# Complexity-ML/complexity-tokenizer

Hardware: AMD Instinct MI355X
Metric: MB/s raw UTF-8 encoded (encode_batch), 50k ByteLevel BPE, 1/2/4/8 MI355X (higher is better)
Workload: dtype u8

## Files before the change

### complexity-tokenizer_amd/complexity_tokenizer/__init__.py

```python
from __future__ import annotations

import ctypes
import gc
import os

import numpy as np

from . import _native as _n
from . import _fast

__version__ = "0.3.3"
__all__ = ["Tokenizer", "Trainer", "Encoding", "BatchEncoding", "PanicException", "UnsupportedConfigError",
           "DeviceError", "__version__"]


class PanicException(BaseException):
    """Raised where the reference raises pyo3_runtime.PanicException (a Rust panic), e.g. a
    merge rank that indexes past the list of valid merges (reference src/bpe.rs:141)."""


class UnsupportedConfigError(NotImplementedError):
    """tokenizer.json selects a component outside the ByteLevel-BPE encode path."""


# ... 209 lines not shown
            buf = ctypes.create_string_buffer(1024)
            rc = _n.lib.ctok_special_token(self._h, i, buf, 1024, ctypes.byref(n), ctypes.byref(tid))
            if rc != _n.CTOK_OK:
                _raise(rc)
            if n.value > 1024:
                buf = ctypes.create_string_buffer(n.value)
                _n.lib.ctok_special_token(self._h, i, buf, n.value, ctypes.byref(n), ctypes.byref(tid))
            out[buf.raw[:n.value].decode("utf-8")] = int(tid.value)
        return out

    def num_piece_added_tokens(self) -> int:
        return int(_n.lib.ctok_num_piece_added_tokens(self._h))

    @property
    def table_props(self) -> dict:
        tp = _n.TableProps()
        rc = _n.lib.ctok_get_table_props(self._h, int(self.device), ctypes.byref(tp))
        if rc != _n.CTOK_OK:
            _raise(rc)
        return {k: None if getattr(tp, k) < 0 else bool(getattr(tp, k)) for k, _ in tp._fields_}

    def encode_packed(self, text: np.ndarray, off: np.ndarray, timing: bool = False):
        text = np.ascontiguousarray(text, dtype=np.uint8)
        off = np.ascontiguousarray(off, dtype=np.uint64)
        n_docs = len(off) - 1
        if n_docs < 0:
            raise ValueError("offsets must hold n_docs + 1 entries")
        n_bytes = int(off[-1]) if n_docs >= 0 else 0
        if len(text) < n_bytes:
            raise ValueError("text shorter than offsets[-1]")
        cap = int(n_bytes + n_docs + 16)
        while True:
            ids = np.empty(max(cap, 1), dtype=np.uint32)
            tok_off = np.empty(n_docs + 1, dtype=np.uint64)
            ex = self._host_exec(timing)
# ... 395 lines not shown
```

### complexity-tokenizer_amd/complexity_tokenizer/_native.py

```python
from __future__ import annotations

import ctypes
import os

_HERE = os.path.dirname(os.path.abspath(__file__))
LIB_PATH = os.environ.get("CTOK_LIB", os.path.join(_HERE, "libctok.so"))

if not os.path.exists(LIB_PATH):
    raise ImportError(
        "complexity_tokenizer: native library not found at %s -- build it with "
        "`make -C complexity-tokenizer_amd/csrc` (or `python -c 'import __graft_entry__ as g; g.build()'`)" % LIB_PATH)


def _share_torch_hip_runtime():
    if os.environ.get("CTOK_NO_TORCH_HIP"):
        return
    try:
        import importlib.util
        spec = importlib.util.find_spec("torch")
    except (ImportError, ValueError):
        return
    if spec is None or not spec.origin:
        return
    path = os.path.join(os.path.dirname(spec.origin), "lib", "libamdhip64.so")
# ... 68 lines not shown

class PadOpts(ctypes.Structure):
    _fields_ = [("flags", ctypes.c_uint32), ("pad_id", ctypes.c_uint32), ("max_length", ctypes.c_uint64)]


class Tables(ctypes.Structure):
    _fields_ = [("vocab", ctypes.c_char_p), ("vocab_off", ctypes.c_void_p), ("vocab_id", ctypes.c_void_p),
                ("n_vocab", ctypes.c_uint64), ("merge_left", ctypes.c_void_p), ("merge_right", ctypes.c_void_p),
                ("n_merges", ctypes.c_uint64), ("added", ctypes.c_char_p), ("added_off", ctypes.c_void_p),
                ("added_id", ctypes.c_void_p), ("added_flags", ctypes.c_void_p), ("n_added", ctypes.c_uint64),
                ("nfc", ctypes.c_int), ("add_prefix_space", ctypes.c_int)]


class TableProps(ctypes.Structure):
    _fields_ = [(k, ctypes.c_int) for k in ("narrow", "compact", "short_packed", "ids16", "dev_narrow",
                                            "dev_short_packed", "last_rec16", "last_wire16")]


class TrainerConfig(ctypes.Structure):
    _fields_ = [("vocab_size", ctypes.c_uint64), ("min_frequency", ctypes.c_uint32),
                ("min_word_length", ctypes.c_uint64), ("inl_alpha", ctypes.c_float), ("inl_beta", ctypes.c_float),
                ("inl_gate", ctypes.c_float), ("inl_mu_target", ctypes.c_float),
                ("inl_velocity_max", ctypes.c_float), ("inl_beta_max", ctypes.c_float),
                ("special", ctypes.c_char_p), ("special_off", ctypes.POINTER(ctypes.c_uint64)),
                ("n_special", ctypes.c_uint64), ("device", ctypes.c_int)]


class TrainerCountStats(ctypes.Structure):
    _fields_ = [("pieces", ctypes.c_uint64), ("words", ctypes.c_uint64), ("unique_words", ctypes.c_uint64),
                ("chunks", ctypes.c_uint64), ("host_chunks", ctypes.c_uint64), ("rerun_chunks", ctypes.c_uint64),
                ("bytes_d2h", ctypes.c_uint64), ("ms_device", ctypes.c_double), ("ms_host", ctypes.c_double)]
# ... 67 lines not shown
```

### complexity-tokenizer_amd/csrc/ctok_host.cpp

```cpp
#include <emmintrin.h>
#include <sched.h>
#include <hip/hip_runtime.h>

#include <algorithm>
#include <atomic>
#include <chrono>
#include <cstdio>
#include <cstring>
#include <exception>
#include <fstream>
#include <functional>
#include <map>
#include <memory>
#include <mutex>
#include <sstream>
#include <thread>
#include <string>
#include <string_view>
#include <unordered_map>
#include <unordered_set>
#include <vector>

#include "../../include/ctok.h"
#include "ctok_internal.h"
// ... 1326 lines not shown
  tb.comp_val = ds->comp_val.p;
  tb.n_comp = CT_COMP_N;
  tb.bytemap_alnum = ds->alnum.p;
  tb.at_bytes = ds->at_bytes.p;
  tb.at_off = ds->at_off.p;
  tb.at_id = ds->at_id.p;
  tb.at_flags = ds->at_flags.p;
  tb.n_at = (uint32_t)t->at_id.size();
  tb.proper = (t->proper && !getenv("CTOK_FORCE_IMPROPER")) ? 1 : 0;
  tb.compact = t->compact ? 1 : 0;
  tb.narrow = (t->narrow && !getenv("CTOK_FORCE_WIDE_SLOTS")) ? 1 : 0;
  {
    const char* pk = getenv("CTOK_SHORT_PACKED");
    tb.short_packed = (tb.narrow && t->short_packed && !(pk && atoi(pk) == 0)) ? 1 : 0;
  }
  tb.all_bytes = std::all_of(t->byte2id, t->byte2id + 256, [](int32_t v) { return v >= 0; }) ? 1 : 0;
  tb.dbg = getenv("CTOK_DBG_MODE") ? (uint32_t)atoi(getenv("CTOK_DBG_MODE")) : 0;
  DeviceState* r = ds.get();
  t->devs[device] = std::move(ds);
  return r;
}

bool debug_sync() {
  static int v = -1;
  if (v < 0) v = getenv("CTOK_DEBUG_SYNC") ? 1 : 0;
  return v == 1;
}

#define STEP(name, x)                                                                    \
  do {                                                                                   \
// ... 336 lines not shown
    ds->lw_pos.ensure(n_long + 8);
    ds->lwn.ensure(n_long + 8);
    ds->scan_tmp2.ensure(scan_tmp_elems(n_long + 1) + 64);
    w.long_pos = ds->long_pos.p;
    w.lw_pos = ds->lw_pos.p;
    STEP("long_prep", launch_long_prep(w, tb, ds->side, n_long, ds->lwn.p, (uint32_t*)ds->scan_tmp2.p,
                                       ds->scan_tmp2.cap * 2));
    HIPTRY(hipMemcpyAsync((void*)tot, ds->long_pos.p + n_long, 4, hipMemcpyDeviceToHost, ds->side));
    HIPTRY(hipMemcpyAsync((void*)(tot + 1), ds->lw_pos.p + n_long, 4, hipMemcpyDeviceToHost, ds->side));
    HIPTRY(hipEventRecord(ds->ev_tot, ds->side));
  }
  const uint32_t c3n = seg_cnt[kCtrC3Count];
  const bool c3_sparse = c3n != 0 && c3n <= c3_limit && c3n <= w.c3_max;
  const char* ov_var = getenv("CTOK_OVERLAP");
  const int overlap = ov_var ? atoi(ov_var) : kOverlapDefault;
  const bool mid_side = overlap >= 1 && seg_cnt[0] == 0;
  ds->last_mid_side = mid_side;
  STEP("bpe_mid", launch_bpe_class(w, tb, 2, mid_side ? ds->side : s, lx(8, 10)));
  if (c3_sparse) STEP("bpe_c3_sparse", launch_c3_sparse(w, tb, c3n, s, lx(-1, 9)));
  else STEP("bpe_c3", launch_bpe_class(w, tb, 4, s, lx(-1, 9)));
  if (!spec_fail1 && n_long) {
    for (;;) {
      const hipError_t e = hipEventQuery(ds->ev_tot);
      if (e == hipSuccess) break;
      if (e != hipErrorNotReady) throw_err(CTOK_E_DEVICE, std::string("hipEventQuery: ") + hipGetErrorString(e));
    }
    const bool any_gmem = tot[1] != 0;
    ds->lids.ensure((uint64_t)tot[0] + 64);
    ds->lw.ensure(4 * (uint64_t)tot[1] + 64);
    w.lids = ds->lids.p;
    w.lw = ds->lw.p;
    STEP("bpe_long", launch_bpe_long(w, tb, ds->side, n_long, seg_cnt[kCtrAnyC3] != 0 && !c3_sparse, any_gmem));
  }
  if (n_long || mid_side) {
    HIPTRY(hipEventRecord(ds->ev_join, ds->side));
    HIPTRY(hipStreamWaitEvent(s, ds->ev_join, 0));
  }
  const bool dropped_pass = tb.n_at == 0 && !tb.all_bytes;
  STEP("bpe_dropped", launch_bpe_class(w, tb, 3, s, lx(5, -1)));
  static const bool copy_res = getenv("CTOK_COPY_RESULTS") != nullptr;
  w.host_res = copy_res ? nullptr : ds->host_dev;
  STEP("emit", launch_emit(w, d_ids, ids_cap, d_tok_off, s, st != nullptr, seg_cnt[kCtrEmptyDocs] != 0,
                           lx(3, -1), lx(-1, 6)));
  if (!w.host_res) {
    HIPTRY(hipMemcpyAsync(ds->host, d_tok_off + n_docs, 8, hipMemcpyDeviceToHost, s));
    HIPTRY(hipMemcpyAsync(ds->host + 1, ds->counters.p, kNumCounters * 4, hipMemcpyDeviceToHost, s));
  }
  Laps laps;
  int lap[11];
  if (tm) {
    hipEvent_t* e = ds->ev;
    const bool passes = tb.n_at == 0;
    lap[0] = laps.add(e[0], e[1]);
    lap[1] = laps.add(e[7], e[1]);
    lap[2] = laps.add(e[1], e[2]);
    lap[3] = !passes ? -1 : mid_side ? laps.add(e[2], e[10]) : laps.add(e[8], e[10]);
    lap[4] = passes ? laps.add(e[2], e[9]) : -1;
    lap[5] = laps.add(e[1], e[2]);
    lap[6] = passes ? laps.add(e[1], e[10]) : -1;
    lap[7] = passes ? laps.add(e[1], e[9]) : -1;
    lap[8] = laps.add(e[1], e[dropped_pass ? 5 : 3]);
    lap[9] = laps.add(e[3], e[6]);
    lap[10] = laps.add(e[0], e[6]);
  }
  HP(5);
  spin_sync(ds, s, [&] { laps.poll(); });
  HP(6);
  laps.finish();
  HP(7);
  uint64_t ntok = ((volatile uint64_t*)ds->host)[0];
  if (w.wgrec) {
    std::vector<uint64_t> r(kWgRecWords);
    HIPTRY(hipMemcpy(r.data(), w.wgrec, kWgRecWords * 8, hipMemcpyDeviceToHost));
    uint64_t t0 = ~0ull;
// ... 656 lines not shown
int ctok_special_token(const ctok* t, uint64_t i, char* buf, size_t cap, size_t* len, uint32_t* id) {
  if (!t || !len || !id) return fail(CTOK_E_ARG, "null argument");
  if (i >= t->special.size()) return fail(CTOK_E_ARG, "index out of range");
  const auto& e = t->special[i];
  *len = e.first.size();
  *id = e.second;
  if (buf && cap) memcpy(buf, e.first.data(), std::min(cap, e.first.size()));
  return CTOK_OK;
}

uint64_t ctok_num_piece_added_tokens(const ctok* t) { return t ? t->at_id.size() : 0; }

int ctok_get_table_props(const ctok* tc, int device, ctok_table_props* out) {
  if (!tc || !out) return fail(CTOK_E_ARG, "null argument");
  ctok* t = const_cast<ctok*>(tc);
  *out = ctok_table_props{t->narrow, t->compact, t->short_packed, t->ids16, -1, -1, -1, -1};
  std::lock_guard<std::mutex> lk(t->dev_mu);
  auto it = t->devs.find(device);
  if (it != t->devs.end()) {
    const DeviceState& ds = *it->second;
    out->dev_narrow = (int)ds.t.narrow;
    out->dev_short_packed = (int)ds.t.short_packed;
    out->last_rec16 = ds.last_rec16;
    out->last_wire16 = ds.last_wire16;
  }
  return CTOK_OK;
}

int ctok_piece_can_contain(const uint8_t* raw, size_t len) {
  if (!raw && len) return fail(CTOK_E_ARG, "null argument");
  return can_occur_in_piece(std::string((const char*)raw, len)) ? 1 : 0;
}

uint64_t ctok_ids_bound(const ctok*, uint64_t n_bytes, uint64_t n_docs) { return 3 * n_bytes + n_docs + 16; }

int ctok_device_count(void) {
  int n = 0;
  if (hipGetDeviceCount(&n) != hipSuccess) return 0;
  return n;
// ... 566 lines not shown
```

### complexity-tokenizer_amd/csrc/ctok_internal.h

```cpp
#pragma once
#include <hip/hip_runtime.h>

#include <cstdint>

namespace ctok_dev {

constexpr uint64_t kEmpty = ~0ull;
constexpr uint32_t kIdBits = 21;
constexpr uint64_t kKeyMask = (1ull << 42) - 1;
constexpr uint32_t kNoRank = 0x3FFFFFu;
constexpr uint32_t kMaxId = (1u << kIdBits) - 2;
constexpr uint32_t kPanicVal = kNoRank - 1;

constexpr uint32_t kErrPanic = 1u;

constexpr int kTileWords = 62;
constexpr int kTile = kTileWords * 64;
constexpr int kTileSlots = 4096;
constexpr int kSegWaves = 4;
constexpr int kSegUnroll = 4;
constexpr int kShortMax = 32;
constexpr int kMedMax = 64;
constexpr uint32_t kCap0 = kTile, kCap1 = (kTile + 8) / 9, kCap2 = (kTile + 16) / 17, kCap3 = (kTile + 32) / 33;
constexpr uint32_t kCap0Lean = 1040;
constexpr int kNumClasses = 4;
constexpr int kNumCounters = 32;
constexpr int kC3Shards = 64;
constexpr int kCounterWords = kNumCounters + kC3Shards;
__host__ __device__ constexpr int ctr_stat(int c) { return c < 3 ? 6 + 2 * c : 16; }
__host__ __device__ constexpr int ctr_chunk(int c) { return c < 3 ? 13 + c : 18; }
constexpr int kCtrAnyMid = 19;
constexpr int kCtrAnyC3 = 20;
constexpr int kCtrEmptyDocs = 21;
constexpr int kCtrC3Count = 22;
constexpr int kCtrC3Take = 23;
constexpr uint32_t kC3SparseDefault = 65536;
constexpr uint32_t kWgRecWords = 4 * 1024 * 4;
constexpr int kOverlapDefault = 1;
constexpr int kCtrSink = 31;
constexpr int kCtrOverflow = 25;
constexpr int kCtrLongIds = 26;
constexpr int kCtrLwWords = 27;
constexpr int kCtrRounds = 29;
constexpr int kLhBuckets = 65;
constexpr int kLhHist = 0, kLhScan = 80, kLhFill = 160, kLhTake = 240, kLhWords = 320;
__host__ __device__ inline uint32_t long_bucket(uint32_t n) { return n > 4096 ? 0u : 64u - (n - 1) / 64; }
__host__ __device__ inline uint32_t list_entry(uint32_t sl, uint32_t o, uint32_t n) { return sl | (o << 12) | (n << 24); }
__host__ __device__ inline uint32_t ent_len(uint32_t e) { return (e >> 24) & 127u; }
__host__ __device__ inline uint32_t ent_ord(uint32_t e) { return (e >> 12) & 0xFFFu; }
__host__ __device__ inline uint32_t long_ord(uint64_t e) { return (uint32_t)(e >> 32) & 0xFFFu; }
__host__ __device__ inline uint32_t long_len(uint64_t e) { return (uint32_t)(e >> 44) & 0x7FFFFu; }

// ... 84 lines not shown
  const uint32_t* comp_val;
  uint32_t n_comp;
  const uint8_t* bytemap_alnum;
  const uint8_t* at_bytes;
  const uint32_t* at_off;
  const uint32_t* at_id;
  const uint8_t* at_flags;
  uint32_t n_at;
  uint32_t proper;
  const uint32_t* eager;
  uint32_t window;
  const uint32_t* wmeta;
  uint32_t compact;
  uint32_t narrow;
  uint32_t short_packed;
  uint32_t dbg;
  uint32_t all_bytes;
};

struct Work {
  const uint8_t* text;
  uint32_t n_bytes;
  const uint64_t* doc_off;
  uint32_t n_docs;
  uint32_t* tfirst;
  uint32_t* pbits;
  uint32_t n_words;
  uint32_t n_tiles;
  uint32_t n_cus;
  uint32_t nfc_watch;
  uint32_t* nfc_bits;
  uint32_t mid_wide;
  uint32_t short_wgs;
// ... 147 lines not shown
```

### complexity-tokenizer_amd/csrc/kernels.hip

```cpp
#include <hip/hip_ext.h>
#include <hip/hip_runtime.h>

#include <algorithm>
#include <mutex>
#include <type_traits>

#include "ctok_internal.h"
#include "merge16_hd.h"
#include "seg_lane.h"

namespace ctok_dev {

#define HIPCHK(x) do { hipError_t e_ = (x); if (e_ != hipSuccess) return e_; } while (0)

template <typename F, typename... A>
static void launch_lx(const Lx& x, F k, dim3 grid, dim3 block, uint32_t lds, hipStream_t s, A... a) {
  if (x.start || x.stop)
    hipExtLaunchKernelGGL(k, grid, block, lds, s, x.start, x.stop, 0u, a...);
  else
    hipLaunchKernelGGL(k, grid, block, lds, s, a...);
}

constexpr uint32_t kNone = 0xFFFFFFFFu;
constexpr uint32_t kDead = 0xFFFFFFFFu;
// ... 1213 lines not shown
__device__ __forceinline__ void lds8_store_packed(const uint32_t (&T)[8], const uint32_t (&R)[8], lds_u32* s_key,
                                                  lds_u16* s_tok) {
  if constexpr (K0 < K1) {
    s_key[K0 * NT + threadIdx.x] = m16::lds8_key<K0>(R);
    s_tok[K0 * NT + threadIdx.x] = (uint16_t)m16::half<K0>(T);
    lds8_store_packed<K0 + 1, K1, NT>(T, R, s_key, s_tok);
  }
}
template <int K0, int K1>
__device__ __forceinline__ void store_packed_ids(const uint32_t (&T)[8], uint32_t m, uint32_t* out) {
  if constexpr (K0 < K1) {
    if ((uint32_t)K0 < m) out[K0] = m16::half<K0>(T);
    store_packed_ids<K0 + 1, K1>(T, m, out);
  }
}

template <uint32_t SORTCAP, int KT = 64>
struct PassLds {
  uint32_t pre[KT + 1], tsum[KT], tbase[KT], stat[2], bcnt[4], bfill[4], chunk, take, next;
  uint16_t perm[SORTCAP];
};

template <int N, bool COMPACT, bool HOT, uint32_t NT, uint32_t SORTCAP, bool L8 = false, int KT = 64, bool PK = false,
          typename Load>
__device__ __forceinline__ void class_pass(const Work& w, const Tables& t, const PairLds& P, const int32_t* s_b2id,
                                           PassLds<SORTCAP, KT>& S, bool& loaded, Load&& load,
                                           lds_u32* s_key = nullptr, lds_u16* s_tok = nullptr) {
  using LC = LdsClass<N>;
  constexpr int K = KT;
  static_assert(KT <= (int)NT, "a thread per chunk tile");
  const uint32_t tid = threadIdx.x;
  uint32_t* err = &w.counters[2];
  const uint32_t* list = class_list<N>(w);
  const uint32_t cap = class_cap<N>(w);
  const uint32_t* counts = w.tcls + (size_t)LC::cls * w.n_tiles;
  uint32_t st_bytes = 0, st_ids = 0;
  if (tid < 2) S.stat[tid] = 0;
  constexpr uint32_t blo = N == 8 ? 1 : N / 2 + 1, bw = N == 64 ? 8 : N == 32 ? 4 : 2;
  auto bucket = [&](uint32_t n) { return min(3u, (n - blo) / bw); };
  __syncthreads();
  uint32_t take = 1;
  const uint32_t U = w.unit;
  for (;;) {
    if (tid == 0) {
      S.chunk = atomicAdd(&w.counters[ctr_chunk(LC::cls)], take);
// ... 44 lines not shown
      }
      __syncthreads();
    }
    auto entry = [&](uint32_t i, uint32_t& kt) {
      const uint32_t q = sorted ? (uint32_t)S.perm[i] : i;
      kt = tile_of<K>(S.pre, q);
      return list[(size_t)(c0 + kt) * cap + (q - S.pre[kt])];
    };
    auto start_of = [&](uint32_t e, uint32_t kt) { return (c0 + kt) * kTile + (e & 0xFFFu); };
    auto body = [&](uint32_t e, uint32_t kt, const uint32_t* wv, auto&& hook) {
        const uint32_t tile = c0 + kt;
        const uint32_t s = tile * kTile + (e & 0xFFFu);
        const uint32_t o = ent_ord(e);
        const uint32_t n = ent_len(e);
        if constexpr (PK) {
          static_assert(N == 16 && L8 && COMPACT, "the packed tier is the 9..16 B pass's, ahead of merge_lds8, on compact tables");
          uint32_t T[8], R[8], bytes[N];
          bool missing = false;
#pragma unroll
          for (int k = 0; k < N; k++) bytes[k] = byte_of(wv[k >> 2], k);
#pragma unroll
          for (int d = 0; d < 8; d++) {
            const int32_t i0 = s_b2id[bytes[2 * d]], i1 = s_b2id[bytes[2 * d + 1]];
            missing |= (((uint32_t)(2 * d) < n) & (i0 < 0)) | (((uint32_t)(2 * d + 1) < n) & (i1 < 0));
            T[d] = m16::pack2((uint32_t)i0, (uint32_t)i1);
          }
          if (missing) {
            hook();
            const uint32_t mi = atomicAdd(&w.counters[4], 1u);
            if (mi < w.mid_cap)
              w.mid_list[mi] = (uint64_t)s | ((uint64_t)o << 32) | ((uint64_t)n << 48);
            else
              atomicOr(&w.counters[kCtrOverflow], 1u);
            return;
          }
          {
            uint32_t v[N];
#pragma unroll
            for (int k = 0; k < N - 1; k++) v[k] = t.pair0[(bytes[k] << 8) | bytes[k + 1]];
            v[N - 1] = kNoRank;
#pragma unroll
            for (int k = 0; k < N - 1; k++) v[k] = (uint32_t)k + 1 < n ? v[k] : kNoRank;
#pragma unroll
            for (int d = 0; d < 8; d++) R[d] = m16::pack2(v[2 * d], v[2 * d + 1]);
          }
          uint32_t m = n;
          Lookup16<HOT> lk{t, P, err};
          const bool more = m16::tier(T, R, m, 8u, lk);
          hook();
          uint32_t pos = 0;
          auto out_of = [&](uint32_t mm) {
            pos = atomicAdd(&S.tsum[kt], mm);
            return w.scratch + (size_t)tile * kTileSlots + pos;
          };
          if (more) {
            lds8_store_packed<0, 8, NT>(T, R, s_key, s_tok);
            m = merge_lds8_run<COMPACT, HOT, NT>(t, P, m, s_key, s_tok, err, out_of);
          } else {
            store_packed_ids<0, N>(T, m, out_of(m));
          }
          CTOK_CHECK_REC(m >= 1 && m <= n && pos + m <= (uint32_t)kTileSlots && o < (uint32_t)kTileSlots,
                         "[ctok check] packed class pass tile %u: record m=%u n=%u pos=%u ordinal=%u\n", tile, m, n, pos, o);
          w.mrec[(size_t)tile * kTileSlots + o] = rec_short(m, pos);
          st_bytes += n;
          st_ids += m;
          return;
        }
        uint32_t tk[N], rk[N];
        bool missing = false;
        {
#pragma unroll
          for (int k = 0; k < N; k++) {
            const int32_t id = s_b2id[byte_of(wv[k >> 2], k)];
            missing |= ((uint32_t)k < n) & (id < 0);
            tk[k] = (uint32_t)id;
          }
        }
// ... 67 lines not shown
      };
      constexpr int kPw = N / 4;
      uint32_t e0 = 0, kt0 = 0, e1 = 0, kt1 = 0;
      uint32_t d0[kPw + 1], sh0 = 0;
#pragma unroll
      for (int k = 0; k <= kPw; k++) d0[k] = 0;
      const uint32_t last = (w.n_bytes - 1) & ~3u;
      auto issue_words = [&](uint32_t s) {
        const uint32_t a0 = s & ~3u;
#pragma unroll
        for (int k = 0; k <= kPw; k++) d0[k] = *reinterpret_cast<const uint32_t*>(w.text + min(a0 + 4 * k, last));
        sh0 = s & 3u;
      };
      auto hook = [&]() {
        static_assert(kPw <= 8, "hook operands");
        if constexpr (kPw == 2) asm volatile("" ::"v"(d0[0]), "v"(d0[1]), "v"(d0[2]), "v"(e1));
        else if constexpr (kPw == 4)
          asm volatile("" ::"v"(d0[0]), "v"(d0[1]), "v"(d0[2]), "v"(d0[3]), "v"(d0[4]), "v"(e1));
        else
          asm volatile("" ::"v"(d0[0]), "v"(d0[1]), "v"(d0[2]), "v"(d0[3]), "v"(d0[4]), "v"(d0[5]), "v"(d0[6]),
                       "v"(d0[7]), "v"(d0[8]), "v"(e1));
      };
      uint32_t b0 = take();
      uint32_t b1 = b0 < E ? take() : E;
      if (b0 + lane < E) {
        e0 = entry(b0 + lane, kt0);
        issue_words(start_of(e0, kt0));
      }
      if (b1 + lane < E) e1 = entry(b1 + lane, kt1);
      hook();
      while (b0 < E) {
        const uint32_t i = b0 + lane;
        const uint32_t b2 = b1 < E ? take() : E;
        const uint32_t e = e0, kt = kt0;
        uint32_t wv[kPw];
#pragma unroll
        for (int k = 0; k < kPw; k++) wv[k] = __builtin_amdgcn_alignbyte(d0[k + 1], d0[k], sh0);
        e0 = e1;
        kt0 = kt1;
        if (b1 + lane < E) issue_words(start_of(e0, kt0));
        if (b2 + lane < E) e1 = entry(b2 + lane, kt1);
        b0 = b1;
        b1 = b2;
        if (i < E) body(e, kt, wv, hook);
        else hook();
      }
    }
    tile_share_flush<K>(w, c0, tb1, S.tsum, S.tbase, LC::cls);
    const uint32_t units = (w.n_tiles + U - 1) / U, next = S.chunk + S.take;
    const uint32_t share = next < units ? (units - next) / gridDim.x : 0u;
    take = min(min((uint32_t)K / U, max(1u, share)), N <= 16 ? 64u : max(1u, (2 * NT * S.take + E) / (E + 1)));
    __syncthreads();
  }
#pragma unroll
  for (int o = 32; o > 0; o >>= 1) {
    st_bytes += (uint32_t)__shfl_xor((int)st_bytes, o, 64);
    st_ids += (uint32_t)__shfl_xor((int)st_ids, o, 64);
  }
  if ((tid & 63) == 0) {
    atomicAdd(&S.stat[0], st_bytes);
// ... 8 lines not shown
}


#ifndef CTOK_SHORT_NT
#define CTOK_SHORT_NT 1024
#endif
#ifndef CTOK_SHORT_SORTCAP
#define CTOK_SHORT_SORTCAP 7168
#endif
template <bool NARROW> struct ShortCfg {
  static constexpr uint32_t NT = NARROW ? CTOK_SHORT_NT : 1024;
  static constexpr uint32_t SORTCAP = NARROW ? CTOK_SHORT_SORTCAP : kSortCap;
};
constexpr int kShortKT = 64;

template <bool COMPACT, bool NARROW, bool PK16 = false>
__global__ __launch_bounds__(1024) void k_bpe_short(Work w, Tables t, uint32_t passes) {
  static_assert((NARROW && COMPACT) || !PK16, "the packed tier needs the narrow tables and compact values");
  if (w.report && blockIdx.x == 0 && threadIdx.x < 64) write_report(w);
  if (spec_failed(w)) return;
  constexpr uint32_t NT = ShortCfg<NARROW>::NT;
  extern __shared__ __attribute__((aligned(16))) uint4 s_img[];
  __shared__ int32_t s_b2id[256];
  __shared__ PassLds<ShortCfg<NARROW>::SORTCAP, kShortKT> S;
  __shared__ uint32_t s_key[NARROW ? 8 * NT : 1];
  __shared__ uint16_t s_tok[NARROW ? 8 * NT : 1];
  const uint32_t tid = threadIdx.x;
  const uint4* img = NARROW ? t.lds16_image : t.lds_image;
  auto load = [&] {
    for (uint32_t i = tid; i < kLdsImageBytes / 16; i += NT) s_img[i] = img[i];
    for (uint32_t i = tid; i < 256; i += NT) s_b2id[i] = t.byte2id[i];
  };
  bool loaded = false;
  const PairLds P{(const lds_u64*)s_img, (const lds_u32*)(s_img + kHotBuckets)};
  lds_u32* sk = (lds_u32*)s_key;
  lds_u16* st = (lds_u16*)s_tok;
  WgRec::begin(w.wgrec, 0);
  if (passes & 1u)
    class_pass<8, COMPACT, true, NT, ShortCfg<NARROW>::SORTCAP, NARROW, kShortKT>(w, t, P, s_b2id, S, loaded, load, sk, st);
  if (passes & 2u)
    class_pass<16, COMPACT, true, NT, ShortCfg<NARROW>::SORTCAP, NARROW, kShortKT, PK16>(w, t, P, s_b2id, S, loaded, load, sk, st);
  WgRec::end(w.wgrec, 0, loaded ? 1u : 0u);
}


template <bool COMPACT, bool NARROW>
__device__ __forceinline__ uint32_t merge_wave64(const Tables& t, const PairLds& P, uint32_t& tok, uint32_t rk,
                                                 uint64_t& lv, uint32_t* err) {
  const uint32_t lane = threadIdx.x & 63;
  for (;;) {
    const uint32_t best = wave_min_full_u32((rk << 6) | lane);
    const uint32_t r = best >> 6, bi = best & 63u;
    if (r == kNoRank) break;
    const uint32_t nid = COMPACT ? r : uni(t.rank_newid[r]);
    const uint64_t right = lv & ~((2ull << bi) - 1ull);
    const uint32_t p = (uint32_t)__builtin_ctzll(right);
// ... 82 lines not shown
  WgRec::begin(w.wgrec, 3);
  extern __shared__ __attribute__((aligned(16))) uint4 s_dyn[];
  __shared__ int32_t s_b2id[256];
  const uint32_t tid = threadIdx.x;
  const uint4* img = NARROW ? t.lds16_image : t.lds_image;
  for (uint32_t i = tid; i < kLdsImageBytes / 16; i += 64 * kSparseWaves) s_dyn[i] = img[i];
  for (uint32_t i = tid; i < 256; i += 64 * kSparseWaves) s_b2id[i] = t.byte2id[i];
  __syncthreads();
  const PairLds P{(const lds_u64*)s_dyn, (const lds_u32*)(s_dyn + kHotBuckets)};
  sparse_c3<COMPACT, NARROW>(w, t, P, s_b2id, n);
  __syncthreads();
  WgRec::end(w.wgrec, 3, 1);
}


template <int CLS> struct MidCfg { static constexpr int KT = 256; };

template <bool COMPACT, int CLS, bool NARROW, uint32_t NT = 512>
__global__ __launch_bounds__(NT) void k_bpe_mid(Work w, Tables t) {
  if (spec_failed(w)) return;
  constexpr int KT = MidCfg<CLS>::KT;
  extern __shared__ __attribute__((aligned(16))) uint4 s_img[];
  __shared__ int32_t s_b2id[256];
  __shared__ PassLds<kSortCap, KT> S;
  __shared__ uint32_t s_key[NARROW ? 8 * NT : 1];
  __shared__ uint16_t s_tok[NARROW ? 8 * NT : 1];
  if constexpr (CLS == 2) WgRec::begin(w.wgrec, 1);
  if (w.counters[CLS == 2 ? kCtrAnyMid : kCtrAnyC3] == 0) {
    if constexpr (CLS == 2) WgRec::end(w.wgrec, 1, 0);
    return;
  }
  __shared__ uint32_t s_left;
  if (threadIdx.x == 0)
    s_left = (uint64_t)__atomic_load_n(&w.counters[ctr_chunk(CLS)], __ATOMIC_RELAXED) * w.unit < w.n_tiles;
  __syncthreads();
  if (!s_left) {
    if constexpr (CLS == 2) WgRec::end(w.wgrec, 1, 0);
    return;
  }
  const uint32_t tid = threadIdx.x;
  const uint4* img = NARROW ? t.lds16_image : t.lds_image;
  for (uint32_t i = tid; i < kLdsImageBytes / 16; i += NT) s_img[i] = img[i];
  for (uint32_t i = tid; i < 256; i += NT) s_b2id[i] = t.byte2id[i];
  bool loaded = true;
  const PairLds P{(const lds_u64*)s_img, (const lds_u32*)(s_img + kHotBuckets)};
  class_pass<CLS == 2 ? 32 : 64, COMPACT, true, NT, kSortCap, NARROW, KT>(w, t, P, s_b2id, S, loaded, [] {},
                                                                         (lds_u32*)s_key, (lds_u16*)s_tok);
  if constexpr (CLS == 2) WgRec::end(w.wgrec, 1, 1);
}

struct LdsAttr {
  std::mutex mu;
  uint64_t done = 0;
};
static hipError_t lds_attr_once(LdsAttr& a, const void* fn, size_t bytes) {
  int dev = 0;
  HIPCHK(hipGetDevice(&dev));
  const uint64_t bit = dev < 64 ? 1ull << dev : 0ull;
  std::lock_guard<std::mutex> lk(a.mu);
  if (a.done & bit) return hipSuccess;
  HIPCHK(hipFuncSetAttribute(fn, hipFuncAttributeMaxDynamicSharedMemorySize, (int)bytes));
  a.done |= bit;
  return hipSuccess;
}

template <bool C, int CLS, bool NW>
static hipError_t launch_mid_t(const Work& w, const Tables& t, hipStream_t s, const Lx& x) {
  static LdsAttr attr;
  HIPCHK(lds_attr_once(attr, (const void*)k_bpe_mid<C, CLS, NW>, kLdsImageBytes));
  if (!w.n_tiles) return hipSuccess;
  const uint32_t grid = min((w.n_tiles + w.unit - 1) / w.unit, w.n_cus);
  if constexpr (CLS == 2) {
    if (w.mid_wide) {
      static LdsAttr attr768;
      HIPCHK(lds_attr_once(attr768, (const void*)k_bpe_mid<C, CLS, NW, 768>, kLdsImageBytes));
      launch_lx(x, k_bpe_mid<C, CLS, NW, 768>, grid, 768, kLdsImageBytes, s, w, t);
      return hipGetLastError();
    }
  }
  launch_lx(x, k_bpe_mid<C, CLS, NW>, grid, 512, kLdsImageBytes, s, w, t);
  return hipGetLastError();
}
template <bool C, int CLS>
static hipError_t launch_mid(const Work& w, const Tables& t, hipStream_t s, const Lx& x = {}) {
  return t.narrow ? launch_mid_t<C, CLS, true>(w, t, s, x) : launch_mid_t<C, CLS, false>(w, t, s, x);
}

template <bool C, bool NW, bool PK = false>
static hipError_t launch_short_t(const Work& w, const Tables& t, hipStream_t s, const Lx& x) {
  static LdsAttr attr;
  HIPCHK(lds_attr_once(attr, (const void*)k_bpe_short<C, NW, PK>, kLdsImageBytes));
  if (!w.n_tiles) return hipSuccess;
  const uint32_t grid = min((w.n_tiles + w.unit - 1) / w.unit, w.short_wgs ? min(w.short_wgs, w.n_cus) : w.n_cus);
  if (t.dbg == 30) {
    k_bpe_short<C, NW, PK><<<grid, ShortCfg<NW>::NT, kLdsImageBytes, s>>>(w, t, 1u);
    k_bpe_short<C, NW, PK><<<grid, ShortCfg<NW>::NT, kLdsImageBytes, s>>>(w, t, 2u);
  } else {
    launch_lx(x, k_bpe_short<C, NW, PK>, grid, ShortCfg<NW>::NT, kLdsImageBytes, s, w, t, 3u);
  }
  return hipGetLastError();
}
template <bool C>
static hipError_t launch_short(const Work& w, const Tables& t, hipStream_t s, const Lx& x) {
  if constexpr (C) {
    if (t.narrow && t.short_packed) return launch_short_t<true, true, true>(w, t, s, x);
  }
  return t.narrow ? launch_short_t<C, true>(w, t, s, x) : launch_short_t<C, false>(w, t, s, x);
}

template <bool C, bool NW>
static hipError_t launch_sparse_t(const Work& w, const Tables& t, uint32_t n_pieces, hipStream_t s, const Lx& x) {
  static LdsAttr attr;
  HIPCHK(lds_attr_once(attr, (const void*)k_bpe_sparse<C, NW>, kLdsImageBytes));
  const uint32_t grid = std::max(1u, std::min((n_pieces + kSparseWaves - 1) / kSparseWaves, w.n_cus));
  launch_lx(x, k_bpe_sparse<C, NW>, grid, 64 * kSparseWaves, kLdsImageBytes, s, w, t, n_pieces);
  return hipGetLastError();
}

hipError_t launch_c3_sparse(const Work& w, const Tables& t, uint32_t n_pieces, hipStream_t s, Lx x) {
// ... 1944 lines not shown
```

### include/ctok.h

```cpp
#ifndef CTOK_H
#define CTOK_H

#include <stddef.h>
#include <stdint.h>

#ifdef __cplusplus
extern "C" {
#endif

typedef struct ctok ctok;

enum {
  CTOK_OK = 0,
  CTOK_E_IO = -1,
  CTOK_E_PARSE = -2,
  CTOK_E_UNSUPPORTED = -3,
  CTOK_E_ARG = -4,
  CTOK_E_CAPACITY = -5,
  CTOK_E_PANIC = -6,
  CTOK_E_DEVICE = -7,
  CTOK_E_NOTFOUND = -8
};

const char* ctok_last_error(void);
// ... 29 lines not shown
void ctok_destroy(ctok* tok);

uint64_t ctok_vocab_size(const ctok* tok);
int ctok_token_to_id(const ctok* tok, const char* token, size_t len, uint32_t* id);
int ctok_id_to_token(const ctok* tok, uint32_t id, char* buf, size_t cap, size_t* len);
uint64_t ctok_num_special_tokens(const ctok* tok);
int ctok_special_token(const ctok* tok, uint64_t i, char* buf, size_t cap, size_t* len, uint32_t* id);

uint64_t ctok_num_piece_added_tokens(const ctok* tok);
int ctok_piece_can_contain(const uint8_t* raw, size_t len);

typedef struct ctok_table_props {
  int narrow, compact, short_packed, ids16;
  int dev_narrow, dev_short_packed;
  int last_rec16, last_wire16;
} ctok_table_props;
int ctok_get_table_props(const ctok* tok, int device, ctok_table_props* out);

typedef struct ctok_exec {
  int device;
  void* stream;
  uint32_t flags;
  const int* devices;
  int n_devices;
  uint32_t chunk_mb;
  uint32_t host_threads;
} ctok_exec;

#define CTOK_F_TIMING 1u

// ... 97 lines not shown
```

Before: 168,800.

## Fold 17..32 B BPE pass into short kernel with packed register merge tier

```diff
diff --git a/complexity-tokenizer_amd/complexity_tokenizer/__init__.py b/complexity-tokenizer_amd/complexity_tokenizer/__init__.py
--- a/complexity-tokenizer_amd/complexity_tokenizer/__init__.py
+++ b/complexity-tokenizer_amd/complexity_tokenizer/__init__.py
@@ -247,11 +247,13 @@
 
     @property
     def table_props(self) -> dict:
-        tp = _n.TableProps()
+        tp = _n.TableProps(dev_mid_packed=-1)
         rc = _n.lib.ctok_get_table_props(self._h, int(self.device), ctypes.byref(tp))
         if rc != _n.CTOK_OK:
             _raise(rc)
-        return {k: None if getattr(tp, k) < 0 else bool(getattr(tp, k)) for k, _ in tp._fields_}
+        d = {k: None if getattr(tp, k) < 0 else bool(getattr(tp, k)) for k, _ in tp._fields_}
+        d["dev_mid_packed"] = None if tp.dev_mid_packed < 0 else int(tp.dev_mid_packed)
+        return d
 
     def encode_packed(self, text: np.ndarray, off: np.ndarray, timing: bool = False):
         text = np.ascontiguousarray(text, dtype=np.uint8)
diff --git a/complexity-tokenizer_amd/complexity_tokenizer/_native.py b/complexity-tokenizer_amd/complexity_tokenizer/_native.py
--- a/complexity-tokenizer_amd/complexity_tokenizer/_native.py
+++ b/complexity-tokenizer_amd/complexity_tokenizer/_native.py
@@ -106,7 +106,7 @@
 
 class TableProps(ctypes.Structure):
     _fields_ = [(k, ctypes.c_int) for k in ("narrow", "compact", "short_packed", "ids16", "dev_narrow",
-                                            "dev_short_packed", "last_rec16", "last_wire16")]
+                                            "dev_short_packed", "last_rec16", "last_wire16", "dev_mid_packed")]
 
 
 class TrainerConfig(ctypes.Structure):
diff --git a/complexity-tokenizer_amd/csrc/ctok_host.cpp b/complexity-tokenizer_amd/csrc/ctok_host.cpp
--- a/complexity-tokenizer_amd/csrc/ctok_host.cpp
+++ b/complexity-tokenizer_amd/csrc/ctok_host.cpp
@@ -1364,6 +1364,13 @@
     const char* pk = getenv("CTOK_SHORT_PACKED");
     tb.short_packed = (tb.narrow && t->short_packed && !(pk && atoi(pk) == 0)) ? 1 : 0;
   }
+  {
+    const char* mp = getenv("CTOK_MID_PACKED");
+    const int want = mp ? atoi(mp) : kMidPackedDefault;
+    uint32_t v = (tb.narrow && tb.compact && t->short_packed && want > 0) ? (want >= 2 ? 2u : 1u) : 0u;
+    if (v == 2 && !tb.short_packed) v = 1;
+    tb.mid_packed = v;
+  }
   tb.all_bytes = std::all_of(t->byte2id, t->byte2id + 256, [](int32_t v) { return v >= 0; }) ? 1 : 0;
   tb.dbg = getenv("CTOK_DBG_MODE") ? (uint32_t)atoi(getenv("CTOK_DBG_MODE")) : 0;
   DeviceState* r = ds.get();
@@ -1730,11 +1737,14 @@
   const bool c3_sparse = c3n != 0 && c3n <= c3_limit && c3n <= w.c3_max;
   const char* ov_var = getenv("CTOK_OVERLAP");
   const int overlap = ov_var ? atoi(ov_var) : kOverlapDefault;
-  const bool mid_side = overlap >= 1 && seg_cnt[0] == 0;
+  const bool folded = nt && mid_folded(tb, seg_cnt[0]);
+  const bool mid_side = !folded && overlap >= 1 && seg_cnt[0] == 0;
   ds->last_mid_side = mid_side;
-  STEP("bpe_mid", launch_bpe_class(w, tb, 2, mid_side ? ds->side : s, lx(8, 10)));
-  if (c3_sparse) STEP("bpe_c3_sparse", launch_c3_sparse(w, tb, c3n, s, lx(-1, 9)));
-  else STEP("bpe_c3", launch_bpe_class(w, tb, 4, s, lx(-1, 9)));
+  if (!folded) STEP("bpe_mid", launch_bpe_class(w, tb, 2, mid_side ? ds->side : s, lx(8, 10)));
+  const bool c3_side = folded && overlap >= 1 && (c3n != 0 || seg_cnt[kCtrAnyC3] != 0);
+  hipStream_t c3s = c3_side ? ds->side : s;
+  if (c3_sparse) STEP("bpe_c3_sparse", launch_c3_sparse(w, tb, c3n, c3s, lx(-1, 9)));
+  else STEP("bpe_c3", launch_bpe_class(w, tb, 4, c3s, lx(-1, 9)));
   if (!spec_fail1 && n_long) {
     for (;;) {
       const hipError_t e = hipEventQuery(ds->ev_tot);
@@ -1748,7 +1758,7 @@
     w.lw = ds->lw.p;
     STEP("bpe_long", launch_bpe_long(w, tb, ds->side, n_long, seg_cnt[kCtrAnyC3] != 0 && !c3_sparse, any_gmem));
   }
-  if (n_long || mid_side) {
+  if (n_long || mid_side || c3_side) {
     HIPTRY(hipEventRecord(ds->ev_join, ds->side));
     HIPTRY(hipStreamWaitEvent(s, ds->ev_join, 0));
   }
@@ -1770,10 +1780,10 @@
     lap[0] = laps.add(e[0], e[1]);
     lap[1] = laps.add(e[7], e[1]);
     lap[2] = laps.add(e[1], e[2]);
-    lap[3] = !passes ? -1 : mid_side ? laps.add(e[2], e[10]) : laps.add(e[8], e[10]);
+    lap[3] = !passes || folded ? -1 : mid_side ? laps.add(e[2], e[10]) : laps.add(e[8], e[10]);
     lap[4] = passes ? laps.add(e[2], e[9]) : -1;
     lap[5] = laps.add(e[1], e[2]);
-    lap[6] = passes ? laps.add(e[1], e[10]) : -1;
+    lap[6] = passes && !folded ? laps.add(e[1], e[10]) : -1;
     lap[7] = passes ? laps.add(e[1], e[9]) : -1;
     lap[8] = laps.add(e[1], e[dropped_pass ? 5 : 3]);
     lap[9] = laps.add(e[3], e[6]);
@@ -2460,7 +2470,7 @@
 int ctok_get_table_props(const ctok* tc, int device, ctok_table_props* out) {
   if (!tc || !out) return fail(CTOK_E_ARG, "null argument");
   ctok* t = const_cast<ctok*>(tc);
-  *out = ctok_table_props{t->narrow, t->compact, t->short_packed, t->ids16, -1, -1, -1, -1};
+  *out = ctok_table_props{t->narrow, t->compact, t->short_packed, t->ids16, -1, -1, -1, -1, -1};
   std::lock_guard<std::mutex> lk(t->dev_mu);
   auto it = t->devs.find(device);
   if (it != t->devs.end()) {
@@ -2469,6 +2479,7 @@
     out->dev_short_packed = (int)ds.t.short_packed;
     out->last_rec16 = ds.last_rec16;
     out->last_wire16 = ds.last_wire16;
+    out->dev_mid_packed = (int)ds.t.mid_packed;
   }
   return CTOK_OK;
 }
diff --git a/complexity-tokenizer_amd/csrc/ctok_internal.h b/complexity-tokenizer_amd/csrc/ctok_internal.h
--- a/complexity-tokenizer_amd/csrc/ctok_internal.h
+++ b/complexity-tokenizer_amd/csrc/ctok_internal.h
@@ -36,6 +36,7 @@
 constexpr int kCtrC3Take = 23;
 constexpr uint32_t kC3SparseDefault = 65536;
 constexpr uint32_t kWgRecWords = 4 * 1024 * 4;
+constexpr int kMidPackedDefault = 2;
 constexpr int kOverlapDefault = 1;
 constexpr int kCtrSink = 31;
 constexpr int kCtrOverflow = 25;
@@ -150,9 +151,14 @@
   uint32_t compact;
   uint32_t narrow;
   uint32_t short_packed;
+  uint32_t mid_packed;
   uint32_t dbg;
   uint32_t all_bytes;
 };
+
+__host__ __device__ inline bool mid_folded(const Tables& t, uint32_t long_pieces) {
+  return t.mid_packed == 2 && t.short_packed && t.n_at == 0 && long_pieces == 0;
+}
 
 struct Work {
   const uint8_t* text;
diff --git a/complexity-tokenizer_amd/csrc/kernels.hip b/complexity-tokenizer_amd/csrc/kernels.hip
--- a/complexity-tokenizer_amd/csrc/kernels.hip
+++ b/complexity-tokenizer_amd/csrc/kernels.hip
@@ -7,6 +7,7 @@
 
 #include "ctok_internal.h"
 #include "merge16_hd.h"
+#include "merge32_hd.h"
 #include "seg_lane.h"
 
 namespace ctok_dev {
@@ -1251,6 +1252,13 @@
     store_packed_ids<K0 + 1, K1>(T, m, out);
   }
 }
+template <int K0, int K1>
+__device__ __forceinline__ void store_packed_ids(const uint32_t (&T)[16], uint32_t m, uint32_t* out) {
+  if constexpr (K0 < K1) {
+    if ((uint32_t)K0 < m) out[K0] = m32::half<K0>(T);
+    store_packed_ids<K0 + 1, K1>(T, m, out);
+  }
+}
 
 template <uint32_t SORTCAP, int KT = 64>
 struct PassLds {
@@ -1259,13 +1267,14 @@
 };
 
 template <int N, bool COMPACT, bool HOT, uint32_t NT, uint32_t SORTCAP, bool L8 = false, int KT = 64, bool PK = false,
-          typename Load>
+          bool LA = true, typename Load, int SKT>
 __device__ __forceinline__ void class_pass(const Work& w, const Tables& t, const PairLds& P, const int32_t* s_b2id,
-                                           PassLds<SORTCAP, KT>& S, bool& loaded, Load&& load,
+                                           PassLds<SORTCAP, SKT>& S, bool& loaded, Load&& load,
                                            lds_u32* s_key = nullptr, lds_u16* s_tok = nullptr) {
   using LC = LdsClass<N>;
   constexpr int K = KT;
   static_assert(KT <= (int)NT, "a thread per chunk tile");
+  static_assert(KT <= SKT, "the shared scratch holds the pass's chunk");
   const uint32_t tid = threadIdx.x;
   uint32_t* err = &w.counters[2];
   const uint32_t* list = class_list<N>(w);
@@ -1340,13 +1349,15 @@
         const uint32_t o = ent_ord(e);
         const uint32_t n = ent_len(e);
         if constexpr (PK) {
-          static_assert(N == 16 && L8 && COMPACT, "the packed tier is the 9..16 B pass's, ahead of merge_lds8, on compact tables");
-          uint32_t T[8], R[8], bytes[N];
+          static_assert((N == 16 || N == 32) && L8 && COMPACT,
+                        "the packed tiers are the 9..16 B and 17..32 B passes', ahead of merge_lds8, on compact tables");
+          constexpr int ND = N / 2;
+          uint32_t T[ND], R[ND], bytes[N];
           bool missing = false;
 #pragma unroll
           for (int k = 0; k < N; k++) bytes[k] = byte_of(wv[k >> 2], k);
 #pragma unroll
-          for (int d = 0; d < 8; d++) {
+          for (int d = 0; d < ND; d++) {
             const int32_t i0 = s_b2id[bytes[2 * d]], i1 = s_b2id[bytes[2 * d + 1]];
             missing |= (((uint32_t)(2 * d) < n) & (i0 < 0)) | (((uint32_t)(2 * d + 1) < n) & (i1 < 0));
             T[d] = m16::pack2((uint32_t)i0, (uint32_t)i1);
@@ -1368,25 +1379,42 @@
 #pragma unroll
             for (int k = 0; k < N - 1; k++) v[k] = (uint32_t)k + 1 < n ? v[k] : kNoRank;
 #pragma unroll
-            for (int d = 0; d < 8; d++) R[d] = m16::pack2(v[2 * d], v[2 * d + 1]);
+            for (int d = 0; d < ND; d++) R[d] = m16::pack2(v[2 * d], v[2 * d + 1]);
           }
           uint32_t m = n;
           Lookup16<HOT> lk{t, P, err};
-          const bool more = m16::tier(T, R, m, 8u, lk);
-          hook();
           uint32_t pos = 0;
           auto out_of = [&](uint32_t mm) {
             pos = atomicAdd(&S.tsum[kt], mm);
             return w.scratch + (size_t)tile * kTileSlots + pos;
           };
-          if (more) {
-            lds8_store_packed<0, 8, NT>(T, R, s_key, s_tok);
-            m = merge_lds8_run<COMPACT, HOT, NT>(t, P, m, s_key, s_tok, err, out_of);
+          if constexpr (N == 32) {
+            bool more = m32::tier(T, R, m, 16u, lk);
+            uint32_t T8[8], R8[8];
+            m32::low_half(T, T8);
+            m32::low_half(R, R8);
+            if (more) more = m16::tier(T8, R8, m, 8u, lk);
+            hook();
+            if (more) {
+              lds8_store_packed<0, 8, NT>(T8, R8, s_key, s_tok);
+              m = merge_lds8_run<COMPACT, HOT, NT>(t, P, m, s_key, s_tok, err, out_of);
+            } else if (m > 16) {
+              store_packed_ids<0, N>(T, m, out_of(m));
+            } else {
+              store_packed_ids<0, 16>(T8, m, out_of(m));
+            }
           } else {
-            store_packed_ids<0, N>(T, m, out_of(m));
+            const bool more = m16::tier(T, R, m, 8u, lk);
+            hook();
+            if (more) {
+              lds8_store_packed<0, 8, NT>(T, R, s_key, s_tok);
+              m = merge_lds8_run<COMPACT, HOT, NT>(t, P, m, s_key, s_tok, err, out_of);
+            } else {
+              store_packed_ids<0, N>(T, m, out_of(m));
+            }
           }
           CTOK_CHECK_REC(m >= 1 && m <= n && pos + m <= (uint32_t)kTileSlots && o < (uint32_t)kTileSlots,
-                         "[ctok check] packed class pass tile %u: record m=%u n=%u pos=%u ordinal=%u\n", tile, m, n, pos, o);
+                         "[ctok check] packed class pass N=%d tile %u: record m=%u n=%u pos=%u ordinal=%u\n", N, tile, m, n, pos, o);
           w.mrec[(size_t)tile * kTileSlots + o] = rec_short(m, pos);
           st_bytes += n;
           st_ids += m;
@@ -1484,7 +1512,8 @@
       };
       auto hook = [&]() {
         static_assert(kPw <= 8, "hook operands");
-        if constexpr (kPw == 2) asm volatile("" ::"v"(d0[0]), "v"(d0[1]), "v"(d0[2]), "v"(e1));
+        if constexpr (!LA) asm volatile("" ::"v"(e1));
+        else if constexpr (kPw == 2) asm volatile("" ::"v"(d0[0]), "v"(d0[1]), "v"(d0[2]), "v"(e1));
         else if constexpr (kPw == 4)
           asm volatile("" ::"v"(d0[0]), "v"(d0[1]), "v"(d0[2]), "v"(d0[3]), "v"(d0[4]), "v"(e1));
         else
@@ -1493,27 +1522,44 @@
       };
       uint32_t b0 = take();
       uint32_t b1 = b0 < E ? take() : E;
-      if (b0 + lane < E) {
-        e0 = entry(b0 + lane, kt0);
-        issue_words(start_of(e0, kt0));
-      }
-      if (b1 + lane < E) e1 = entry(b1 + lane, kt1);
-      hook();
-      while (b0 < E) {
-        const uint32_t i = b0 + lane;
-        const uint32_t b2 = b1 < E ? take() : E;
-        const uint32_t e = e0, kt = kt0;
-        uint32_t wv[kPw];
-#pragma unroll
-        for (int k = 0; k < kPw; k++) wv[k] = __builtin_amdgcn_alignbyte(d0[k + 1], d0[k], sh0);
-        e0 = e1;
-        kt0 = kt1;
-        if (b1 + lane < E) issue_words(start_of(e0, kt0));
-        if (b2 + lane < E) e1 = entry(b2 + lane, kt1);
-        b0 = b1;
-        b1 = b2;
-        if (i < E) body(e, kt, wv, hook);
-        else hook();
+      if constexpr (LA) {
+        if (b0 + lane < E) {
+          e0 = entry(b0 + lane, kt0);
+          issue_words(start_of(e0, kt0));
+        }
+        if (b1 + lane < E) e1 = entry(b1 + lane, kt1);
+        hook();
+        while (b0 < E) {
+          const uint32_t i = b0 + lane;
+          const uint32_t b2 = b1 < E ? take() : E;
+          const uint32_t e = e0, kt = kt0;
+          uint32_t wv[kPw];
+#pragma unroll
+          for (int k = 0; k < kPw; k++) wv[k] = __builtin_amdgcn_alignbyte(d0[k + 1], d0[k], sh0);
+          e0 = e1;
+          kt0 = kt1;
+          if (b1 + lane < E) issue_words(start_of(e0, kt0));
+          if (b2 + lane < E) e1 = entry(b2 + lane, kt1);
+          b0 = b1;
+          b1 = b2;
+          if (i < E) body(e, kt, wv, hook);
+          else hook();
+        }
+      } else {
+        if (b0 + lane < E) e1 = entry(b0 + lane, kt1);
+        while (b0 < E) {
+          const uint32_t i = b0 + lane;
+          const uint32_t b2 = b1 < E ? take() : E;
+          const bool live = i < E;
+          const uint32_t e = live ? e1 : 0u, kt = live ? kt1 : 0u;
+          uint32_t wv[kPw];
+          load_words<kPw>(w.text, start_of(e, kt), w.n_bytes, wv);
+          if (b1 + lane < E) e1 = entry(b1 + lane, kt1);
+          b0 = b1;
+          b1 = b2;
+          if (live) body(e, kt, wv, hook);
+          else hook();
+        }
       }
     }
     tile_share_flush<K>(w, c0, tb1, S.tsum, S.tbase, LC::cls);
@@ -1552,15 +1598,19 @@
 };
 constexpr int kShortKT = 64;
 
-template <bool COMPACT, bool NARROW, bool PK16 = false>
+constexpr int kMidKT = 256;
+constexpr uint32_t kFoldSortCut = 3 * (kMidKT - kShortKT) * 4 / 2;
+template <bool COMPACT, bool NARROW, bool PK16 = false, bool PK32 = false>
 __global__ __launch_bounds__(1024) void k_bpe_short(Work w, Tables t, uint32_t passes) {
   static_assert((NARROW && COMPACT) || !PK16, "the packed tier needs the narrow tables and compact values");
+  static_assert(PK16 || !PK32, "the third pass is the packed instance's");
   if (w.report && blockIdx.x == 0 && threadIdx.x < 64) write_report(w);
   if (spec_failed(w)) return;
   constexpr uint32_t NT = ShortCfg<NARROW>::NT;
+  constexpr uint32_t SORTCAP = ShortCfg<NARROW>::SORTCAP - (PK32 ? kFoldSortCut : 0u);
   extern __shared__ __attribute__((aligned(16))) uint4 s_img[];
   __shared__ int32_t s_b2id[256];
-  __shared__ PassLds<ShortCfg<NARROW>::SORTCAP, kShortKT> S;
+  __shared__ PassLds<SORTCAP, PK32 ? kMidKT : kShortKT> S;
   __shared__ uint32_t s_key[NARROW ? 8 * NT : 1];
   __shared__ uint16_t s_tok[NARROW ? 8 * NT : 1];
   const uint32_t tid = threadIdx.x;
@@ -1575,9 +1625,18 @@
   lds_u16* st = (lds_u16*)s_tok;
   WgRec::begin(w.wgrec, 0);
   if (passes & 1u)
-    class_pass<8, COMPACT, true, NT, ShortCfg<NARROW>::SORTCAP, NARROW, kShortKT>(w, t, P, s_b2id, S, loaded, load, sk, st);
+    class_pass<8, COMPACT, true, NT, SORTCAP, NARROW, kShortKT>(w, t, P, s_b2id, S, loaded, load, sk, st);
   if (passes & 2u)
-    class_pass<16, COMPACT, true, NT, ShortCfg<NARROW>::SORTCAP, NARROW, kShortKT, PK16>(w, t, P, s_b2id, S, loaded, load, sk, st);
+    class_pass<16, COMPACT, true, NT, SORTCAP, NARROW, kShortKT, PK16>(w, t, P, s_b2id, S, loaded, load, sk, st);
+  if constexpr (PK32) {
+    if (passes & 4u) {
+      if (tid == 0) S.next = (mid_folded(t, w.counters[0]) && w.counters[kCtrAnyMid] != 0) ? 1u : 0u;
+      __syncthreads();
+      const uint32_t fold = S.next;
+      if (fold)
+        class_pass<32, COMPACT, true, NT, SORTCAP, NARROW, kMidKT, true, false>(w, t, P, s_b2id, S, loaded, load, sk, st);
+    }
+  }
   WgRec::end(w.wgrec, 0, loaded ? 1u : 0u);
 }
 
@@ -1690,10 +1749,11 @@
 }
 
 
-template <int CLS> struct MidCfg { static constexpr int KT = 256; };
-
-template <bool COMPACT, int CLS, bool NARROW, uint32_t NT = 512>
+template <int CLS> struct MidCfg { static constexpr int KT = kMidKT; };
+
+template <bool COMPACT, int CLS, bool NARROW, uint32_t NT = 512, bool PK = false>
 __global__ __launch_bounds__(NT) void k_bpe_mid(Work w, Tables t) {
+  static_assert(!PK || (CLS == 2 && NARROW && COMPACT), "the packed tiers need the narrow tables and compact values");
   if (spec_failed(w)) return;
   constexpr int KT = MidCfg<CLS>::KT;
   extern __shared__ __attribute__((aligned(16))) uint4 s_img[];
@@ -1720,8 +1780,8 @@
   for (uint32_t i = tid; i < 256; i += NT) s_b2id[i] = t.byte2id[i];
   bool loaded = true;
   const PairLds P{(const lds_u64*)s_img, (const lds_u32*)(s_img + kHotBuckets)};
-  class_pass<CLS == 2 ? 32 : 64, COMPACT, true, NT, kSortCap, NARROW, KT>(w, t, P, s_b2id, S, loaded, [] {},
-                                                                         (lds_u32*)s_key, (lds_u16*)s_tok);
+  class_pass<CLS == 2 ? 32 : 64, COMPACT, true, NT, kSortCap, NARROW, KT, PK>(w, t, P, s_b2id, S, loaded, [] {},
+                                                                             (lds_u32*)s_key, (lds_u16*)s_tok);
   if constexpr (CLS == 2) WgRec::end(w.wgrec, 1, 1);
 }
 
@@ -1740,45 +1800,50 @@
   return hipSuccess;
 }
 
-template <bool C, int CLS, bool NW>
+template <bool C, int CLS, bool NW, bool PK = false>
 static hipError_t launch_mid_t(const Work& w, const Tables& t, hipStream_t s, const Lx& x) {
   static LdsAttr attr;
-  HIPCHK(lds_attr_once(attr, (const void*)k_bpe_mid<C, CLS, NW>, kLdsImageBytes));
+  HIPCHK(lds_attr_once(attr, (const void*)k_bpe_mid<C, CLS, NW, 512, PK>, kLdsImageBytes));
   if (!w.n_tiles) return hipSuccess;
   const uint32_t grid = min((w.n_tiles + w.unit - 1) / w.unit, w.n_cus);
   if constexpr (CLS == 2) {
     if (w.mid_wide) {
       static LdsAttr attr768;
-      HIPCHK(lds_attr_once(attr768, (const void*)k_bpe_mid<C, CLS, NW, 768>, kLdsImageBytes));
-      launch_lx(x, k_bpe_mid<C, CLS, NW, 768>, grid, 768, kLdsImageBytes, s, w, t);
+      HIPCHK(lds_attr_once(attr768, (const void*)k_bpe_mid<C, CLS, NW, 768, PK>, kLdsImageBytes));
+      launch_lx(x, k_bpe_mid<C, CLS, NW, 768, PK>, grid, 768, kLdsImageBytes, s, w, t);
       return hipGetLastError();
     }
   }
-  launch_lx(x, k_bpe_mid<C, CLS, NW>, grid, 512, kLdsImageBytes, s, w, t);
+  launch_lx(x, k_bpe_mid<C, CLS, NW, 512, PK>, grid, 512, kLdsImageBytes, s, w, t);
   return hipGetLastError();
 }
 template <bool C, int CLS>
 static hipError_t launch_mid(const Work& w, const Tables& t, hipStream_t s, const Lx& x = {}) {
+  if constexpr (C && CLS == 2) {
+    if (t.narrow && t.mid_packed) return launch_mid_t<true, 2, true, true>(w, t, s, x);
+  }
   return t.narrow ? launch_mid_t<C, CLS, true>(w, t, s, x) : launch_mid_t<C, CLS, false>(w, t, s, x);
 }
 
-template <bool C, bool NW, bool PK = false>
+template <bool C, bool NW, bool PK = false, bool PK32 = false>
 static hipError_t launch_short_t(const Work& w, const Tables& t, hipStream_t s, const Lx& x) {
   static LdsAttr attr;
-  HIPCHK(lds_attr_once(attr, (const void*)k_bpe_short<C, NW, PK>, kLdsImageBytes));
+  HIPCHK(lds_attr_once(attr, (const void*)k_bpe_short<C, NW, PK, PK32>, kLdsImageBytes));
   if (!w.n_tiles) return hipSuccess;
   const uint32_t grid = min((w.n_tiles + w.unit - 1) / w.unit, w.short_wgs ? min(w.short_wgs, w.n_cus) : w.n_cus);
   if (t.dbg == 30) {
-    k_bpe_short<C, NW, PK><<<grid, ShortCfg<NW>::NT, kLdsImageBytes, s>>>(w, t, 1u);
-    k_bpe_short<C, NW, PK><<<grid, ShortCfg<NW>::NT, kLdsImageBytes, s>>>(w, t, 2u);
+    k_bpe_short<C, NW, PK, PK32><<<grid, ShortCfg<NW>::NT, kLdsImageBytes, s>>>(w, t, 1u);
+    k_bpe_short<C, NW, PK, PK32><<<grid, ShortCfg<NW>::NT, kLdsImageBytes, s>>>(w, t, 2u);
+    if (PK32) k_bpe_short<C, NW, PK, PK32><<<grid, ShortCfg<NW>::NT, kLdsImageBytes, s>>>(w, t, 4u);
   } else {
-    launch_lx(x, k_bpe_short<C, NW, PK>, grid, ShortCfg<NW>::NT, kLdsImageBytes, s, w, t, 3u);
+    launch_lx(x, k_bpe_short<C, NW, PK, PK32>, grid, ShortCfg<NW>::NT, kLdsImageBytes, s, w, t, PK32 ? 7u : 3u);
   }
   return hipGetLastError();
 }
 template <bool C>
 static hipError_t launch_short(const Work& w, const Tables& t, hipStream_t s, const Lx& x) {
   if constexpr (C) {
+    if (t.narrow && t.short_packed && t.mid_packed == 2) return launch_short_t<true, true, true, true>(w, t, s, x);
     if (t.narrow && t.short_packed) return launch_short_t<true, true, true>(w, t, s, x);
   }
   return t.narrow ? launch_short_t<C, true>(w, t, s, x) : launch_short_t<C, false>(w, t, s, x);
diff --git a/complexity-tokenizer_amd/csrc/merge32_hd.h b/complexity-tokenizer_amd/csrc/merge32_hd.h
--- /dev/null
+++ b/complexity-tokenizer_amd/csrc/merge32_hd.h
@@ -0,0 +1,85 @@
+#pragma once
+#include "merge16_hd.h"
+
+namespace m32 {
+
+using m16::bfi;
+using m16::kNone;
+using m16::pack2;
+using m16::shr16;
+using m16::umin;
+
+M16_HD uint32_t min_key(const uint32_t (&R)[16]) {
+  uint32_t key = ~0u;
+M16_UNROLL
+  for (int d = 0; d < 16; d++) {
+    key = umin(key, (R[d] << 16) | (uint32_t)(2 * d));
+    key = umin(key, (R[d] & 0xFFFF0000u) | (uint32_t)(2 * d + 1));
+  }
+  return key;
+}
+
+template <class LK>
+M16_HD bool step(uint32_t (&T)[16], uint32_t (&R)[16], uint32_t& m, LK& lk) {
+  const uint32_t key = min_key(R);
+  const uint32_t best = key >> 16, bi = key & 31u;
+  if (best == kNone) return false;
+  const uint32_t nid = lk.new_id(best) & 0xFFFFu;
+  const uint32_t D = bi >> 1;
+  const bool odd = (bi & 1u) != 0;
+  uint32_t S[16];
+M16_UNROLL
+  for (int d = 0; d < 16; d++) S[d] = shr16(d + 1 < 16 ? T[d + 1] : ~0u, T[d]);
+  uint32_t A[17];
+  A[0] = odd ? T[0] : 0u;
+M16_UNROLL
+  for (int d = 1; d < 16; d++) A[d] = odd ? T[d] : S[d - 1];
+  A[16] = odd ? ~0u : S[15];
+  uint32_t L0 = 0, R0 = 0;
+M16_UNROLL
+  for (int d = 0; d < 16; d++) {
+    L0 = D == (uint32_t)d ? A[d] : L0;
+    R0 = D == (uint32_t)d ? A[d + 1] : R0;
+  }
+  const uint32_t L = L0 & 0xFFFFu, Rt = R0 >> 16;
+  const bool has_l = bi > 0, has_r = bi + 2 < m;
+  lk.start(L, nid, Rt, has_l, has_r);
+  const uint32_t Y = odd ? (L | (nid << 16)) : (nid | (R0 & 0xFFFF0000u));
+  const uint32_t mA = odd ? 0xFFFFFFFFu : 0x0000FFFFu, mB = odd ? 0u : 0xFFFF0000u;
+  uint32_t mask[16];
+M16_UNROLL
+  for (int d = 0; d < 16; d++) {
+    const bool right = bi < (uint32_t)(2 * d + 1);
+    T[d] = D == (uint32_t)d ? Y : (right ? S[d] : T[d]);
+    const uint32_t sr = shr16(d + 1 < 16 ? R[d + 1] : ~0u, R[d]);
+    R[d] = right ? sr : R[d];
+    mask[d] = D == (uint32_t)d ? mA : (D == (uint32_t)(d + 1) ? mB : 0u);
+  }
+  m--;
+  uint32_t rl, rr;
+  lk.finish(rl, rr);
+  const uint32_t vv = odd ? pack2(rl, rr) : pack2(rr, rl);
+M16_UNROLL
+  for (int d = 0; d < 16; d++) R[d] = bfi(mask[d], vv, R[d]);
+  return true;
+}
+
+template <class LK>
+M16_HD bool tier(uint32_t (&T)[16], uint32_t (&R)[16], uint32_t& m, uint32_t stop, LK& lk) {
+  for (;;) {
+    if (m <= stop) return true;
+    if (!step(T, R, m, lk)) return false;
+  }
+}
+
+M16_HD void low_half(const uint32_t (&A)[16], uint32_t (&lo)[8]) {
+M16_UNROLL
+  for (int d = 0; d < 8; d++) lo[d] = A[d];
+}
+
+template <int K>
+M16_HD uint32_t half(const uint32_t (&A)[16]) {
+  return (K & 1) ? A[K >> 1] >> 16 : A[K >> 1] & 0xFFFFu;
+}
+
+}
diff --git a/include/ctok.h b/include/ctok.h
--- a/include/ctok.h
+++ b/include/ctok.h
@@ -67,6 +67,7 @@
   int narrow, compact, short_packed, ids16;
   int dev_narrow, dev_short_packed;
   int last_rec16, last_wire16;
+  int dev_mid_packed;
 } ctok_table_props;
 int ctok_get_table_props(const ctok* tok, int device, ctok_table_props* out);
 
```

Measured after the change: 171,800, median of 6. 1.02x the previous value.
